# nianticlabs/acezero

Hardware: AMD Instinct MI355X
Metric: ACE patches/sec (higher is better)
Workload: dtype bf16; 1 GPU; 7-Scenes-chess-like ace_zero mapping step: 8M-patch bf16 feature buffer in HBM, batch 5120 per GPU, default head (1 block, 2 103 300 params), tanh loss, 1cyclepoly AdamW, pose_refinement none; buffer_patches=8000000, batch_per_gpu=5120, global_batch=5120, parallelism=dp1

## Files before the change

acezero_amd/csrc/head_api.hip:

```cpp
#include "head_kernels.hip"
#include "pose_fused.hip"
#include "head_maps.hip"
#include "acez_common.h"
#include "conv_launch.h"
#include <stdlib.h>
#include <string.h>
#include <algorithm>
#include "acez_common.h"
#include <vector>
#include <new>

using namespace acez;

struct StepCarry {
  bool wave_pending = false;
  const int64_t* idx = nullptr;
  int n = 0;
  bool in_alt = false;
  void hold(const int64_t* i, int k, bool alt) { idx = i; n = k; in_alt = alt; }
  void drop_batch() { hold(nullptr, 0, false); }
};

struct acez_trainer {
  char* arena_base = nullptr;
// ... 33 lines not shown
  TrainState* st_infer = nullptr;
  hipStream_t pose_stream = nullptr;
  hipEvent_t ev_begin = nullptr, ev_pose_fwd = nullptr, ev_loss = nullptr, ev_pose_bwd = nullptr;
  GradReduceArgs last_reduce{};
  StepCarry carry;
  SchedConfig sc;
  std::vector<void*> allocs;
  int pose_images = 0;
  float *pa1 = nullptr, *pa2 = nullptr, *pa3 = nullptr, *pr = nullptr, *pf1 = nullptr, *pf2 = nullptr, *pdlt = nullptr, *pose_cur = nullptr;
  float *pdT = nullptr, *pddelta = nullptr, *pdz2 = nullptr, *pdz1 = nullptr, *pdr = nullptr, *pdzc3 = nullptr, *pdzc2 = nullptr, *pdzc1 = nullptr;
  float* pose_wt = nullptr;
  bool pose_fused = true;
  int pose_tile = 4;
  bool pose_wt_valid = false;
  float* row_dT = nullptr;
  int* row_image = nullptr;
  bool profiling = false;
  std::vector<hipEvent_t> ev_pool;
  struct EvUse { int cls, i0, i1, launches; };
  std::vector<EvUse> ev_used;
  size_t ev_next = 0;
  int prof_launches = 0;
  bool seq = true;
  bool f16 = false;
  int last_nblk = 0;
  int n_cus = 0;
  uint32_t* seq_flags = nullptr;
  uint32_t seq_base[64] = {};
  uint32_t* seq_xcc = nullptr;
  int* seq_err = nullptr;
  uint32_t seq_spin_limit = 40000;
  int seq_faults = 0;
  int seq_probe = -1;
  long seq_launches = 0, seq_fault_at = -1;
  bool wgrad_opt = true;
  float* wg_xch = nullptr;
  uint32_t* wg_flags = nullptr;
  uint32_t wg_epoch = 0;
  uint16_t* R0_alt = nullptr;
  int4* batch_meta_alt = nullptr;
  long wgo_fault_at = -1;
  int wgo_fault_mod = 0;
  uint32_t* wg_status = nullptr;
  WgoFaultRec* wg_rec = nullptr;
  int wgo_recovered = 0;
  bool inference_only = false;
  bool sizing = false;
  size_t sized_total = 0;
  unsigned long long* pose_trace = nullptr;
  unsigned long long* wgo_trace = nullptr;
};

enum { KC_SCHED = 0, KC_GATHER, KC_GEMM_FWD, KC_LOSS, KC_GEMM_DGRAD, KC_WGRAD, KC_REDUCE, KC_ADAMW, KC_COUNT };

static int loss_blocks(int n) { return (n + 15) / 16; }
static int gather_blocks(int n) { return (n + 3) / 4 < 1024 ? (n + 3) / 4 : 1024; }

template <class F>
static void with_pose_tile(const acez_trainer* tr, int n_images, F f) {
  if (tr->pose_tile == 16) f(std::integral_constant<int, 16>{}, (n_images + 15) / 16);
  else f(std::integral_constant<int, 4>{}, (n_images + 3) / 4);
}

struct ProfScope {
  acez_trainer* tr; hipStream_t s; int cls; int i0 = -1;
  ProfScope(acez_trainer* t, hipStream_t st, int c) : tr(t), s(st), cls(c) {
// ... 130 lines not shown
  ACEZ_REQUIRE(cfg->schedule >= 0 && cfg->schedule <= 2, "unknown schedule");
  ACEZ_REQUIRE(cfg->loss_type >= 0 && cfg->loss_type <= 4, "unknown loss type");
  ACEZ_REQUIRE(cfg->pose_refinement >= 0 && cfg->pose_refinement <= 2, "pose_refinement must be 0 (none), 1 (naive) or 2 (mlp)");
  ACEZ_REQUIRE(cfg->pose_refinement_ortho == 0 || cfg->pose_refinement_ortho == 1, "pose_refinement_ortho must be 0 (gram-schmidt) or 1 (procrustes)");
  ACEZ_REQUIRE(cfg->pose_refinement == 0 || (params->d_pose_params && params->d_pose_m && params->d_pose_v), "pose refinement needs the pose parameter buffers");
  ACEZ_REQUIRE(cfg->pose_refinement != 2 || params->n_pose_params == ACEZ_POSE_MLP_PARAMS, "mlp: n_pose_params must be ACEZ_POSE_MLP_PARAMS");
  ACEZ_REQUIRE(cfg->pose_refinement != 1 || (params->n_pose_params > 0 && params->n_pose_params % 12 == 0), "naive: n_pose_params must be 12 * n_images");
  ACEZ_REQUIRE(cfg->compute_dtype != ACEZ_DTYPE_FP32, "compute_dtype fp32 (train_ace.py --use_half False) is not implemented: choose ACEZ_DTYPE_BF16 or ACEZ_DTYPE_FP16");
  ACEZ_REQUIRE(cfg->compute_dtype == ACEZ_DTYPE_BF16 || cfg->compute_dtype == ACEZ_DTYPE_FP16, "unknown compute_dtype");
  if (int rc = acez::require_device("the head kernels need a gfx950 GPU")) return rc;
  if (device >= 0) ACEZ_HIP_CHECK(hipSetDevice(device));
  acez_trainer* tr = new (std::nothrow) acez_trainer();
  ACEZ_REQUIRE(tr, "out of host memory");
  ACEZ_HIP_CHECK(hipGetDevice(&tr->device));
  tr->cfg = *cfg;
  tr->f16 = cfg->compute_dtype == ACEZ_DTYPE_FP16;
  if (const char* e = ACEZ_DIAG_ENV("ACEZ_POSE_FUSED")) tr->pose_fused = atoi(e) != 0;
  if (const char* e = ACEZ_DIAG_ENV("ACEZ_POSE_TILE")) tr->pose_tile = atoi(e) == 16 ? 16 : 4;
  if (cfg->pose_refinement != 2) tr->pose_fused = false;
  if (cfg->pose_refinement != 0 && !tr->pose_fused) {
    ACEZ_HIP_CHECK(hipStreamCreateWithFlags(&tr->pose_stream, hipStreamNonBlocking));
    for (hipEvent_t* e : {&tr->ev_begin, &tr->ev_pose_fwd, &tr->ev_loss, &tr->ev_pose_bwd}) ACEZ_HIP_CHECK(hipEventCreateWithFlags(e, hipEventDisableTiming));
  }
  tr->pb = *params;
  tr->nb = cfg->head.num_head_blocks;
  tr->L = 3 + 3 * tr->nb + 2;
  tr->no = cfg->head.use_homogeneous ? 4 : 3;
  tr->n_wide = (int64_t)tr->L * (512 * 512 + 512);
  tr->fc3_off = tr->n_wide;
  tr->n_params = params->n_params;
  tr->fc3_stride = ((int64_t)tr->no * 513 + 3) & ~3LL;
  tr->max_batch = cfg->max_batch;
  if (const char* e = getenv("ACEZ_SEQ")) tr->seq = atoi(e) != 0;
  {
    hipDeviceProp_t prop;
    ACEZ_HIP_CHECK(hipGetDeviceProperties(&prop, tr->device));
    tr->n_cus = prop.multiProcessorCount;
  }
  tr->nslabs = 256 / (16 * tr->L);
  if (tr->nslabs < 1) tr->nslabs = 1;

  int rc = ACEZ_OK;
  const size_t act_bytes = (size_t)tr->max_batch * 512 * sizeof(uint16_t);
  auto A = [&](void** p, size_t bytes) { if (rc == ACEZ_OK) rc = dmalloc(tr, p, bytes); };
  const bool trains = cfg->inference_only == 0;
  tr->inference_only = !trains;
  const int wgo_grid = 256 * ((tr->L + 7) / 8);
  for (int pass = 0; pass < 2; ++pass) {
  tr->sizing = pass == 0;
  A((void**)&tr->Wb, (size_t)tr->L * 262144 * 2);
  A((void**)&tr->WbT, (size_t)tr->L * 262144 * 2);
  A((void**)&tr->W3b, (size_t)tr->no * 512 * 2);
  tr->out.resize(tr->L, nullptr);
  tr->dZ.resize(tr->L, nullptr);
  tr->R.resize(tr->nb + 2, nullptr);
  for (int l = 0; l < tr->L; ++l) { A((void**)&tr->out[l], act_bytes); if (trains) A((void**)&tr->dZ[l], act_bytes); }
  for (int b = 0; b < tr->nb + 2; ++b) A((void**)&tr->R[b], act_bytes);
  const int max_loss_blocks = loss_blocks(tr->max_batch);
  tr->bias_layer_stride = (int64_t)max_loss_blocks * 512;
  if (trains) {
    A((void**)&tr->dR[0], act_bytes);
    A((void**)&tr->dR[1], act_bytes);
    tr->mask_stride = (size_t)((tr->max_batch + 79) / 80) * 4 * 4 * 64;
    A((void**)&tr->maskbits, (size_t)tr->L * tr->mask_stride * sizeof(uint2));
    A((void**)&tr->slabs, (size_t)tr->nslabs * tr->n_wide * sizeof(float));
    A((void**)&tr->fc3_partials, (size_t)max_loss_blocks * tr->fc3_stride * sizeof(float));
// ... 123 lines not shown
  a.Wb = tr->Wb; a.WbT = tr->WbT; a.W3b = tr->W3b;
  for (int l = 0; l < tr->L; ++l) { a.w_off[l] = (int64_t)l * 262656; a.b_off[l] = a.w_off[l] + 262144; }
  a.fc3_off = tr->fc3_off; a.n_fc3 = (int64_t)tr->no * 513; a.n_params = tr->n_params;
  a.n_layers = tr->L; a.no = tr->no; a.st = tr->st;
  a.slabs = nullptr; a.nslabs = 0; a.slab_stride = 0;
  a.fault = tr->seq_err; a.f16 = tr->f16 ? 1 : 0;
  a.layer_lo = 0; a.layer_hi = tr->L;
}

extern "C" int acez_trainer_sync_weights(acez_trainer* tr, void* stream) {
  ACEZ_REQUIRE(tr, "null trainer");
  ACEZ_HIP_CHECK(hipSetDevice(tr->device));
  AdamArgs a;
  fill_adam_args(tr, a);
  const int nblk = tr->L * 64 + (tr->no * 512 + 255) / 256;
  hipLaunchKernelGGL(recast_kernel, dim3(nblk), dim3(256), 0, (hipStream_t)stream, a);
  ACEZ_HIP_CHECK(hipGetLastError());
  tr->pose_wt_valid = false;
  tr->carry.drop_batch();
  return ACEZ_OK;
}

static bool seq_usable(const acez_trainer* tr, int n) {
  const int mtiles = (n + 79) / 80;
  return tr->seq && mtiles <= 64 && 32 * ((mtiles + 7) / 8) <= tr->n_cus;
}

static bool wgrad_opt_usable(const acez_trainer* tr) {
  return tr->wgrad_opt && tr->seq && tr->nslabs == 2 &&
         tr->cfg.pose_refinement == 0 && 256 * ((tr->L + 7) / 8) <= tr->n_cus;
}

template <bool BWD>
static void launch_rowseq(acez_trainer* tr, const std::vector<SeqLayer>& layers, int n, const TrainState* st, hipStream_t s) {
  const int mtiles = (n + 79) / 80;
  for (size_t i0 = 0; i0 < layers.size(); i0 += SEQ_MAX_LAYERS) {
    RowSeqArgs a{};
    const int cnt = (int)std::min<size_t>(SEQ_MAX_LAYERS, layers.size() - i0);
    for (int i = 0; i < cnt; ++i) a.layer[i] = layers[i0 + i];
    a.n_layers = cnt; a.M = n; a.st = st ? st : tr->st_infer; a.flags = tr->seq_flags; a.xcc_dbg = tr->seq_xcc; a.spin_limit = tr->seq_spin_limit;
    for (int mt = 0; mt < 64; ++mt) a.base[mt] = tr->seq_base[mt];
    if (cnt > 1 && tr->seq_launches == tr->seq_fault_at)
      for (int mt = 0; mt < 64; ++mt) a.base[mt] += 1u << 20;
    ++tr->seq_launches;
    if (tr->f16) hipLaunchKernelGGL((rowseq_kernel<BWD, EltF16>), dim3(32 * ((mtiles + 7) / 8)), dim3(512), 0, s, a);
    else hipLaunchKernelGGL(rowseq_kernel<BWD>, dim3(32 * ((mtiles + 7) / 8)), dim3(512), 0, s, a);
    for (int mt = 0; mt < mtiles; ++mt) tr->seq_base[mt] += (uint32_t)(cnt - 1);
    tr->prof_launches += cnt;
  }
}

static uint16_t* launch_forward(acez_trainer* tr, const uint16_t* in0, int n, const TrainState* st, hipStream_t s,
                                std::vector<SeqLayer>* collect = nullptr) {
  ProfScope chain_scope(tr, s, collect ? -1 : KC_GEMM_FWD);
  const float* P = tr->pb.d_params;
  const bool seq = collect || seq_usable(tr, n);
  std::vector<SeqLayer> sq;
  auto mask_out = [&](int l) -> uint2* { return (st && tr->maskbits && l != 3 * (tr->nb + 1) + 1) ? tr->maskbits + (size_t)l * tr->mask_stride : nullptr; };
  auto gemm = [&](int l, const uint16_t* in, uint16_t* out_main, const uint16_t* res, uint16_t* out_aux) {
    if (seq) {
      SeqLayer y{};
      y.In = in; y.W = tr->Wb + (size_t)l * 262144; y.bias = P + (int64_t)l * 262656 + 262144; y.res = res; y.out_main = out_main;
      y.out_aux = out_aux; y.aux_mode = res ? AUX_RESIDUAL : AUX_NONE;
      y.mask_out = mask_out(l);
      sq.push_back(y);
      return;
    }
    RowGemmArgs g{};
    g.In = in; g.W = tr->Wb + (size_t)l * 262144; g.bias = P + (int64_t)l * 262656 + 262144;
    g.add = nullptr; g.mask_out = mask_out(l); g.mask_in = nullptr; g.res = res; g.out_main = out_main; g.out_aux = out_aux;
    g.M = n; g.N = 512; g.K = 512; g.relu = 1; g.aux_mode = res ? AUX_RESIDUAL : AUX_NONE; g.st = st; g.bias_partials = nullptr;
    launch_rowgemm(g, s, tr->f16);
    ++tr->prof_launches;
  };
  const uint16_t* r = in0;
  for (int b = 0; b <= tr->nb; ++b) {
    gemm(3 * b, r, tr->out[3 * b], nullptr, nullptr);
    gemm(3 * b + 1, tr->out[3 * b], tr->out[3 * b + 1], nullptr, nullptr);
    gemm(3 * b + 2, tr->out[3 * b + 1], mask_out(3 * b + 2) ? nullptr : tr->out[3 * b + 2], r, tr->R[b + 1]);
    r = tr->R[b + 1];
// ... 95 lines not shown
}

static void fill_wgrad_args(acez_trainer* tr, WgradArgs& a, int n, const TrainState* st) {
  const int f1 = 3 * (tr->nb + 1), f2 = f1 + 1;
  for (int l = 0; l < tr->L; ++l) {
    a.dZ[l] = tr->dZ[l];
    a.w_off[l] = (int64_t)l * 262656; a.b_off[l] = a.w_off[l] + 262144;
  }
  for (int b = 0; b <= tr->nb; ++b) {
    a.In[3 * b] = tr->R[b]; a.In[3 * b + 1] = tr->out[3 * b]; a.In[3 * b + 2] = tr->out[3 * b + 1];
  }
  a.In[f1] = tr->R[tr->nb + 1]; a.In[f2] = tr->out[f1];
  a.slabs = tr->slabs; a.slab_stride = tr->n_wide; a.M = n; a.nslabs = tr->nslabs; a.n_layers = tr->L; a.st = st; a.zeros = tr->zeros;
}


enum class Flow { Fused, Backward, Update };
enum class Opt { None, WgradOpt, AdamwPose, AdamwNext, AdamwSplitPose, Adamw };
enum class NextAt { None, Loss, Optimiser };

struct StepPlan {
  Flow flow;
  bool begin_launch = false, begin_gathers = false, begin_pose = false;
  NextAt next_at = NextAt::None;
  Opt opt = Opt::None;
};

struct StepRun {
  acez_trainer* tr;
  StepPlan plan;
  const int64_t* idx; int n;
  const int64_t* next; int n_next;
  int nblk;
  hipStream_t s, ps;
  const TrainState* st;
};

static StepPlan plan_step(const acez_trainer* tr, Flow flow, const int64_t* idx, int n, const int64_t* next, int n_next) {
  StepPlan p{flow};
  const bool pf = tr->pose_fused, announced = next && n_next > 0;
  if (flow != Flow::Update) {
    const StepCarry& c = tr->carry;
    const bool have = !c.in_alt && c.idx == idx && c.n == n;
    p.begin_gathers = !have || (!pf && c.wave_pending);
    p.begin_pose = pf;
    p.begin_launch = p.begin_gathers || pf;
    if (flow == Flow::Backward) return p;
  }
  if (flow == Flow::Fused && wgrad_opt_usable(tr)) p.opt = Opt::WgradOpt;
  else if (flow == Flow::Fused && pf) p.opt = Opt::AdamwPose;
  else if (announced && tr->cfg.pose_refinement == 0 && tr->have_buf) p.opt = Opt::AdamwNext;
  else if (tr->cfg.pose_refinement != 0) p.opt = Opt::AdamwSplitPose;
  else p.opt = Opt::Adamw;
  if (announced && (p.opt == Opt::WgradOpt || p.opt == Opt::AdamwPose)) p.next_at = NextAt::Loss;
  else if (p.opt == Opt::AdamwNext || (announced && p.opt == Opt::AdamwSplitPose && pf && tr->have_buf)) p.next_at = NextAt::Optimiser;
  return p;
}

static void wave_ran(acez_trainer* tr) {
  tr->st_cur ^= 1;
  tr->st = tr->st_slot[tr->st_cur];
  tr->carry.wave_pending = false;
}

static void flush_post(acez_trainer* tr, hipStream_t s) {
  if (!tr->carry.wave_pending) return;
// ... 23 lines not shown
  else if (wave)
    hipLaunchKernelGGL(step_begin_kernel, dim3(gblocks + 1), dim3(256), 0, s, (const uint16_t*)tr->buf.d_features, d_indices, tr->R[0], n,
                       post_args(tr), gather_meta(tr));
  else
    hipLaunchKernelGGL(gather_kernel, dim3(gblocks), dim3(256), 0, s, (const uint16_t*)tr->buf.d_features, d_indices, tr->R[0], n, (const TrainState*)tr->st,
                       gather_meta(tr));
  if (wave) wave_ran(tr);
}

static void close_step(acez_trainer* tr, const StepPlan& p) {
  if (tr->carry.in_alt) {
    std::swap(tr->R[0], tr->R0_alt);
    std::swap(tr->batch_meta, tr->batch_meta_alt);
    tr->carry.in_alt = false;
  }
  if (p.opt != Opt::WgradOpt && p.opt != Opt::AdamwNext) tr->carry.wave_pending = true;
}

static void launch_train_loss(const StepRun& r) {
  acez_trainer* tr = r.tr;
  LossArgs a{};
  fill_loss_train(tr, a, tr->out[3 * (tr->nb + 1) + 1], r.idx, r.n, tr->cfg.pose_refinement != 0);
  tr->last_nblk = r.nblk;
  ProfScope ps(tr, r.s, KC_LOSS);
  if (r.plan.next_at != NextAt::Loss) return launch_loss(tr, r.nblk, r.s, a);
  const int gblocks = std::min((r.n_next + 31) / 32, std::max(32, 2 * tr->n_cus - r.nblk));
  GatherMeta gm = gather_meta(tr);
  gm.dst = tr->batch_meta_alt;
  if (tr->f16) hipLaunchKernelGGL((loss_gather_kernel<EltF16, 4>), dim3(r.nblk + gblocks), dim3(256), 0, r.s, a, r.nblk, (const uint16_t*)tr->buf.d_features, r.next, tr->R0_alt, r.n_next, gm);
  else hipLaunchKernelGGL((loss_gather_kernel<EltBf16, 4>), dim3(r.nblk + gblocks), dim3(256), 0, r.s, a, r.nblk, (const uint16_t*)tr->buf.d_features, r.next, tr->R0_alt, r.n_next, gm);
  tr->carry.hold(r.next, r.n_next, true);
}

static void launch_dgrad(acez_trainer* tr, int n, const TrainState* st, hipStream_t s, std::vector<SeqLayer>* collect = nullptr) {
  const int f1 = 3 * (tr->nb + 1), f2 = f1 + 1;
  const bool seq = collect || seq_usable(tr, n);
  std::vector<SeqLayer> sq;
  auto dgrad = [&](int l, int l_out, const uint16_t* add, uint16_t* out_main, uint16_t* out_aux) {
    const uint2* mask = tr->maskbits + (size_t)l_out * tr->mask_stride;
    if (seq) {
      if (add && !out_aux) abort();
      SeqLayer y{};
      y.In = tr->dZ[l]; y.W = tr->WbT + (size_t)l * 262144; y.add = add; y.mask_in = mask; y.out_main = out_main; y.out_aux = out_aux;
      y.bias_partials = tr->bias_partials + (size_t)l_out * tr->bias_layer_stride; y.aux_mode = out_aux ? AUX_UNMASKED : AUX_NONE;
      sq.push_back(y);
      return;
    }
    RowGemmArgs g{};
    g.bias_partials = tr->bias_partials + (size_t)l_out * tr->bias_layer_stride;
    g.In = tr->dZ[l]; g.W = tr->WbT + (size_t)l * 262144; g.bias = nullptr; g.add = add; g.mask_in = mask; g.mask_out = nullptr; g.res = nullptr;
    g.out_main = out_main; g.out_aux = out_aux; g.M = n; g.N = 512; g.K = 512; g.relu = 0;
    g.aux_mode = out_aux ? AUX_UNMASKED : AUX_NONE; g.st = st;
    g.absmax = tr->f16 ? tr->st->dz_absmax_slots : nullptr;
    launch_rowgemm(g, s, tr->f16);
    ++tr->prof_launches;
  };
  ProfScope dchain(tr, s, collect ? -1 : KC_GEMM_DGRAD);
  dgrad(f2, f1, nullptr, tr->dZ[f1], nullptr);
  int cur = 0;
  dgrad(f1, 3 * tr->nb + 2, nullptr, tr->dZ[3 * tr->nb + 2], tr->dR[cur]);
  for (int b = tr->nb; b >= 0; --b) {
    dgrad(3 * b + 2, 3 * b + 1, nullptr, tr->dZ[3 * b + 1], nullptr);
    dgrad(3 * b + 1, 3 * b, nullptr, tr->dZ[3 * b], nullptr);
    if (b > 0) {
      dgrad(3 * b, 3 * (b - 1) + 2, tr->dR[cur], tr->dZ[3 * (b - 1) + 2], tr->dR[cur ^ 1]);
      cur ^= 1;
    }
  }
  if (collect) *collect = sq;
  else if (seq) launch_rowseq<true>(tr, sq, n, st, s);
}

static void launch_weight_grads(acez_trainer* tr, const StepPlan& p, int n, int nblk, const TrainState* st, hipStream_t s) {
  const bool fused = p.flow == Flow::Fused;
  const int f2 = 3 * (tr->nb + 1) + 1;
  {
    GradReduceArgs a{};
    a.slabs = tr->slabs; a.slab_stride = tr->n_wide; a.nslabs = tr->nslabs; a.fc3_partials = tr->fc3_partials;
    a.fc3_stride = tr->fc3_stride; a.stat_partials = tr->stat_partials; a.n_loss_blocks = nblk; a.grad = tr->pb.d_grad;
    a.n_wide = tr->n_wide; a.n_params = tr->n_params; a.st = st;
    a.bias_partials = tr->bias_partials; a.bias_layer_stride = tr->bias_layer_stride; a.n_layers = tr->L;
    a.skip_wide = fused ? 1 : 0;
    a.fault = tr->seq_err;
    for (int l = 0; l < tr->L; ++l) a.bias_count[l] = (l == f2) ? nblk : (n + 79) / 80;
    tr->last_reduce = a;
  }
  {
    WgradArgs a{};
    fill_wgrad_args(tr, a, n, st);
    ProfScope ps(tr, s, KC_WGRAD);
    const int groups = tr->L * tr->nslabs;
    if (p.opt == Opt::WgradOpt) {
      WgradOptArgs o{};
      fill_adam_args(tr, o.ad);
      o.ad.tail = tr->last_reduce;
      o.xch = tr->wg_xch; o.flags = tr->wg_flags; o.spin_limit = tr->seq_spin_limit;
      o.trace = tr->wgo_trace;
      o.target = 2u * ++tr->wg_epoch;
      o.epoch = tr->wg_epoch; o.status = tr->wg_status; o.rec = tr->wg_rec;
      if ((long)tr->wg_epoch - 1 == tr->wgo_fault_at) {
        if (tr->wgo_fault_mod > 0) o.fault_mod = tr->wgo_fault_mod;
        else o.target += 1u << 20;
      }
// ... 68 lines not shown
  }
  default: {
    ProfScope ps(tr, s, KC_ADAMW);
    hipLaunchKernelGGL(adamw_kernel, dim3(n_adam), dim3(256), 0, s, a);
    break;
  }
  }
  close_step(tr, p);
  ACEZ_HIP_CHECK(hipGetLastError());
  return ACEZ_OK;
}

static void pose_fwd_launches(acez_trainer* tr, hipStream_t q) {
  if (tr->cfg.pose_refinement == 2) pose_forward(tr, &tr->st->active, q);
  if (tr->cfg.pose_refinement == 1)
    hipLaunchKernelGGL(pose_compose_kernel, dim3((tr->buf.n_images + 255) / 256), dim3(256), 0, q, (const float*)tr->pa1,
                       (const float*)tr->pb.d_pose_params, 1.0f, tr->pose_cur, tr->buf.n_images, (const int*)&tr->st->active, tr->cfg.pose_refinement_ortho);
}
static void pose_bwd_launches(acez_trainer* tr, int n, hipStream_t q) {
  if (tr->cfg.pose_refinement == 0) return;
  const int I = tr->buf.n_images;
  const int* active = &tr->st->active;
  hipLaunchKernelGGL(pose_grad_reduce2_kernel, dim3((I + 15) / 16), dim3(256), 0, q, (const float*)tr->row_dT, (const int*)tr->row_image, n, tr->pdT, I, active);
  if (tr->cfg.pose_refinement == 2) {
    hipLaunchKernelGGL(pose_mlp_bwd_kernel, dim3((I + PN_IMG - 1) / PN_IMG), dim3(256), 0, q, pose_net_args(tr, active));
    launch_pose_wgrad(tr, active, false, q);
  } else {
    hipLaunchKernelGGL(pose_compose_bwd_kernel, dim3((I + 255) / 256), dim3(256), 0, q, (const float*)tr->pa1, (const float*)tr->pb.d_pose_params, 1.0f,
                       (const float*)tr->pdT, tr->pb.d_grad + tr->n_params + 4, I, active, tr->cfg.pose_refinement_ortho);
  }
}

static StepRun start_run(acez_trainer* tr, Flow flow, const int64_t* idx, int n, const int64_t* next, int n_next, hipStream_t s) {
  return StepRun{tr, plan_step(tr, flow, idx, n, next, n_next), idx, n, next, n_next, loss_blocks(n), s, tr->pose_stream ? tr->pose_stream : s, nullptr};
}

static void launch_chain(const StepRun& r, bool bwd) {
  if (bwd) launch_dgrad(r.tr, r.n, r.st, r.s);
  else launch_forward(r.tr, r.tr->R[0], r.n, r.st, r.s);
}

template <class Chains>
static int run_steps(StepRun* runs, int count, Chains chains) {
  for (int i = 0; i < count; ++i) {
    StepRun& r = runs[i];
    acez_trainer* tr = r.tr;
    tr->last_n = r.n;
    begin_step(tr, r.plan, r.idx, r.n, r.s);
    r.st = tr->st;
    if (r.ps != r.s) {
      ACEZ_HIP_CHECK(hipEventRecord(tr->ev_begin, r.s));
      ACEZ_HIP_CHECK(hipStreamWaitEvent(r.ps, tr->ev_begin, 0));
    }
    if (!tr->pose_fused) pose_fwd_launches(tr, r.ps);
    if (r.ps != r.s) ACEZ_HIP_CHECK(hipEventRecord(tr->ev_pose_fwd, r.ps));
  }
  chains(false);
  for (int i = 0; i < count; ++i) {
    StepRun& r = runs[i];
    acez_trainer* tr = r.tr;
    if (r.ps != r.s) ACEZ_HIP_CHECK(hipStreamWaitEvent(r.s, tr->ev_pose_fwd, 0));
    launch_train_loss(r);
    if (r.ps != r.s) {
      ACEZ_HIP_CHECK(hipEventRecord(tr->ev_loss, r.s));
      ACEZ_HIP_CHECK(hipStreamWaitEvent(r.ps, tr->ev_loss, 0));
    }
    if (!tr->pose_fused) pose_bwd_launches(tr, r.n, r.ps);
    if (r.ps != r.s) ACEZ_HIP_CHECK(hipEventRecord(tr->ev_pose_bwd, r.ps));
  }
  chains(true);
  for (int i = 0; i < count; ++i) {
    StepRun& r = runs[i];
    acez_trainer* tr = r.tr;
    launch_weight_grads(tr, r.plan, r.n, r.nblk, r.st, r.s);
    if (r.ps != r.s) ACEZ_HIP_CHECK(hipStreamWaitEvent(r.s, tr->ev_pose_bwd, 0));
    if (tr->pose_fused && r.plan.flow == Flow::Backward) launch_pose_wgrad(tr, &tr->st->active, false, r.s);
    ACEZ_HIP_CHECK(hipGetLastError());
    if (r.plan.flow == Flow::Fused) {
      const int rc = launch_update(tr, r.plan, r.s, 0, tr->L, r.next, r.n_next);
      if (rc != ACEZ_OK) return rc;
    }
  }
  return ACEZ_OK;
}

static int train_step_impl(acez_trainer* tr, Flow flow, const int64_t* d_indices, int n, void* stream, const int64_t* d_next = nullptr, int n_next = 0) {
  ACEZ_REQUIRE(tr && d_indices, "null pointer");
  ACEZ_REQUIRE(!tr->inference_only, "an inference-only context (acez_train_config.inference_only) cannot train");
  ACEZ_REQUIRE(tr->have_buf, "acez_trainer_set_buffer has not been called");
  ACEZ_REQUIRE(n > 0 && n <= tr->max_batch, "n must be in [1, max_batch]");
  ACEZ_HIP_CHECK(hipSetDevice(tr->device));
  StepRun r = start_run(tr, flow, d_indices, n, d_next, n_next, (hipStream_t)stream);
  return run_steps(&r, 1, [&](bool bwd) { launch_chain(r, bwd); });
}

extern "C" int acez_train_backward(acez_trainer* tr, const int64_t* d_indices, int n, void* stream) {
  return train_step_impl(tr, Flow::Backward, d_indices, n, stream);
}

static int train_update_impl(acez_trainer* tr, void* stream, int layer_lo, int layer_hi, const int64_t* d_next = nullptr, int n_next = 0) {
  ACEZ_REQUIRE(tr, "null trainer");
  ACEZ_REQUIRE(!tr->inference_only, "an inference-only context (acez_train_config.inference_only) cannot train");
  if (layer_hi < 0) layer_hi = tr->L;
  ACEZ_REQUIRE(layer_lo >= 0 && layer_lo <= layer_hi && layer_hi <= tr->L, "layer range out of bounds");
  ACEZ_HIP_CHECK(hipSetDevice(tr->device));
  return launch_update(tr, plan_step(tr, Flow::Update, nullptr, 0, d_next, n_next), (hipStream_t)stream, layer_lo, layer_hi, d_next, n_next);
}

extern "C" int acez_train_update(acez_trainer* tr, void* stream) { return train_update_impl(tr, stream, 0, -1); }
extern "C" int acez_train_update_next(acez_trainer* tr, const int64_t* d_indices_next, int n_next, void* stream) {
  ACEZ_REQUIRE(n_next >= 0 && (!tr || n_next <= tr->max_batch), "n_next must be in [0, max_batch]");
  return train_update_impl(tr, stream, 0, -1, d_indices_next, n_next);
}

extern "C" int acez_train_update_layers(acez_trainer* tr, int layer_lo, int layer_hi, void* stream) {
  return train_update_impl(tr, stream, layer_lo, layer_hi);
}

extern "C" int acez_trainer_export_weights16(acez_trainer* tr, int layer_lo, int layer_hi, void* d_dst, void* stream) {
  ACEZ_REQUIRE(tr && d_dst, "null pointer");
  ACEZ_REQUIRE(layer_lo >= 0 && layer_lo <= layer_hi && layer_hi <= tr->L, "layer range out of bounds");
  if (layer_hi == layer_lo) return ACEZ_OK;
  ACEZ_HIP_CHECK(hipSetDevice(tr->device));
  ACEZ_HIP_CHECK(hipMemcpyAsync(d_dst, tr->Wb + (size_t)layer_lo * 262144, (size_t)(layer_hi - layer_lo) * 262144 * 2, hipMemcpyDeviceToDevice, (hipStream_t)stream));
  return ACEZ_OK;
// ... 230 lines not shown
```

acezero_amd/csrc/head_kernels.hip:

```cpp
#include <hip/hip_runtime.h>
#include <stdint.h>
#include "head_kernels.h"
#include "gemm_common.h"

namespace acez {


template <int GR = 4>
__device__ __forceinline__ void gather_rows(const uint16_t* __restrict__ feat, const int64_t* __restrict__ idx, uint16_t* __restrict__ out, int n,
                                            int wave, int nwaves, int lane, const GatherMeta& meta) {
  const bool held = meta.hold && *meta.hold;
  for (int r0 = wave; r0 < n; r0 += GR * nwaves) {
    int r[GR];
    bool ok[GR];
    int64_t s[GR];
#pragma unroll
    for (int j = 0; j < GR; ++j) { r[j] = r0 + j * nwaves; ok[j] = r[j] < n; s[j] = idx[ok[j] ? r[j] : r0]; }
    uint4 v[GR];
#pragma unroll
    for (int j = 0; j < GR; ++j) v[j] = *reinterpret_cast<const uint4*>(feat + s[j] * 512 + lane * 8);
    int view[GR];
    float2 tp[GR];
    if (meta.dst) {
#pragma unroll
// ... 380 lines not shown
template <bool BIAS_RELU, bool HAS_ADD, bool HAS_MASK, int AUX, class E = EltBf16>
__global__ __launch_bounds__(512) void rowgemm80_kernel(RowGemmArgs a) {
  const int active = a.st ? a.st->active : 1;
  __shared__ __attribute__((aligned(16))) uint16_t smem[RG80_SMEM];
  const int mtiles = (a.M + 79) / 80;
  const int per_xcd = (mtiles + 7) >> 3;
  const int jx = blockIdx.x >> 3;
  const int mt = (blockIdx.x & 7) * per_xcd + (jx >> 2);
  if (mt >= mtiles) return;
  rowgemm80_body<BIAS_RELU, HAS_ADD, HAS_MASK, AUX, false, E>(a, smem, active, mt, (jx & 3) * 128, SeqLink{});
}

struct SeqLayer {
  const uint16_t *In, *W;
  const float* bias;
  const uint16_t *add, *res;
  uint2* mask_out;
  const uint2* mask_in;
  uint16_t *out_main, *out_aux;
  float* bias_partials;
  int aux_mode, pad;
};
constexpr int SEQ_MAX_LAYERS = 8;
struct RowSeqArgs {
  SeqLayer layer[SEQ_MAX_LAYERS];
  int n_layers, M;
  const TrainState* st;
  uint32_t* flags;
  uint32_t base[64];
  uint32_t spin_limit;
  uint32_t* xcc_dbg;
};

template <bool BWD, class E = EltBf16>
__global__ __launch_bounds__(512) void rowseq_kernel(RowSeqArgs a) {
  __shared__ __attribute__((aligned(16))) uint16_t smem[RG80_SMEM_SEQ];
  const int mtiles = (a.M + 79) / 80;
  const int per_xcd = (mtiles + 7) >> 3;
  const int jx = blockIdx.x >> 3;
  const int mt = (blockIdx.x & 7) * per_xcd + (jx >> 2);
  if (mt >= mtiles) return;
  if (a.xcc_dbg && threadIdx.x == 0) {
    const uint32_t xcc = __builtin_amdgcn_s_getreg((3 << 11) | 20) & 15u;
    atomicOr(a.xcc_dbg + (blockIdx.x & 7), 1u << xcc);
    a.xcc_dbg[8 + mt * 4 + (jx & 3)] = xcc;
  }
  if ((a.st && !a.st->active) || a.flags[64 * 32]) {
    if (threadIdx.x == 0) {
      const uint32_t inc = 8u * (uint32_t)(a.n_layers - 1);
      asm volatile("global_atomic_add %0, %1, off" ::"v"(a.flags + mt * 32), "v"(inc) : "memory");
    }
    return;
  }
  const int n0 = (jx & 3) * 128;
  for (int layer = 0; layer < a.n_layers; ++layer) {
    const SeqLayer& y = a.layer[layer];
    RowGemmArgs g;
    g.In = y.In; g.W = y.W; g.bias = y.bias; g.add = y.add; g.mask_out = y.mask_out; g.mask_in = y.mask_in; g.res = y.res; g.out_main = y.out_main; g.out_aux = y.out_aux;
    g.bias_partials = y.bias_partials; g.M = a.M; g.N = 512; g.K = 512; g.relu = BWD ? 0 : 1; g.aux_mode = y.aux_mode; g.st = a.st;
    g.absmax = (BWD && a.st) ? const_cast<uint32_t*>(a.st->dz_absmax_slots) : nullptr;
    SeqLink q;
    q.flag = a.flags + mt * 32; q.target = (a.base[mt] + (uint32_t)layer) * 32u;
    q.first = layer == 0; q.wait = layer > 0; q.signal = layer + 1 < a.n_layers;
    q.next_W = q.signal ? a.layer[layer + 1].W : nullptr;
    q.flag_index = (uint32_t)(mt * 32); q.limit = a.spin_limit;
    if (!BWD) {
      if (y.aux_mode == AUX_RESIDUAL) rowgemm80_body<true, false, false, AUX_RESIDUAL, true, E>(g, smem, 1, mt, n0, q);
      else rowgemm80_body<true, false, false, AUX_NONE, true, E>(g, smem, 1, mt, n0, q);
    } else {
      if (y.add) rowgemm80_body<false, true, true, AUX_UNMASKED, true, E>(g, smem, 1, mt, n0, q);
      else if (y.aux_mode == AUX_UNMASKED) rowgemm80_body<false, false, true, AUX_UNMASKED, true, E>(g, smem, 1, mt, n0, q);
      else rowgemm80_body<false, false, true, AUX_NONE, true, E>(g, smem, 1, mt, n0, q);
    }
  }
}

__global__ __launch_bounds__(512) void seq_probe_kernel(uint32_t* rec , int mtiles) {
  __shared__ __attribute__((aligned(16))) uint16_t smem[RG80_SMEM_SEQ];
  const int per_xcd = (mtiles + 7) >> 3;
  const int jx = blockIdx.x >> 3;
  const int mt = (blockIdx.x & 7) * per_xcd + (jx >> 2);
  if (threadIdx.x == 0) smem[0] = (uint16_t)blockIdx.x;
  __syncthreads();
  if (mt >= mtiles || threadIdx.x != 0) return;
  const uint32_t xcc = __builtin_amdgcn_s_getreg((3 << 11) | 20) & 15u;
  rec[mt * 4 + (jx & 3)] = (xcc << 16) | smem[0];
}

static inline void launch_rowgemm(const RowGemmArgs& g, hipStream_t s, bool f16 = false) {
  const bool br = g.bias != nullptr;
  const int mtiles = (g.M + 79) / 80;
  const dim3 grid(8 * 4 * ((mtiles + 7) / 8));
#define ACEZ_RG(...)                                                                                               \
  do {                                                                                                             \
    if (f16) hipLaunchKernelGGL((rowgemm80_kernel<__VA_ARGS__, EltF16>), grid, dim3(512), 0, s, g);                \
    else hipLaunchKernelGGL((rowgemm80_kernel<__VA_ARGS__>), grid, dim3(512), 0, s, g);                            \
  } while (0)
  if (br && g.aux_mode == AUX_NONE) ACEZ_RG(true, false, false, AUX_NONE);
  else if (br && g.aux_mode == AUX_RESIDUAL) ACEZ_RG(true, false, false, AUX_RESIDUAL);
  else if (!br && g.mask_in && !g.add && g.aux_mode == AUX_NONE) ACEZ_RG(false, false, true, AUX_NONE);
  else if (!br && g.mask_in && !g.add && g.aux_mode == AUX_UNMASKED) ACEZ_RG(false, false, true, AUX_UNMASKED);
  else if (!br && g.mask_in && g.add && g.aux_mode == AUX_UNMASKED) ACEZ_RG(false, true, true, AUX_UNMASKED);
  else if (!br && g.mask_in && g.add && g.aux_mode == AUX_NONE) ACEZ_RG(false, true, true, AUX_NONE);
  else abort();
#undef ACEZ_RG
}

// ... 1222 lines not shown
    if (threadIdx.x < 64) {
      if (a.slabs) {
        sched_post_wave(p.src, p.st, p.c, p.grad_stats, p.inv_global_batch, p.log_loss, p.log_inl, p.log_cap, p.fault, p.stat_partials, p.n_loss_blocks, &a.tail);
      } else {
        sched_post_wave(p.src, p.st, p.c, p.grad_stats, p.inv_global_batch, p.log_loss, p.log_inl, p.log_cap, p.fault, p.stat_partials, p.n_loss_blocks);
      }
    }
    return;
  }
  adamw_body(a, b - gblocks - 1, tileT);
}

__device__ double det_cos_pi(double x) {
  const double PI = 3.14159265358979323846;
  const double y = (x - 0.5) * PI;
  const double y2 = y * y;
  double term = y, sum = y;
  for (int k = 1; k <= 11; ++k) {
    term = -term * y2 / (double)((2 * k) * (2 * k + 1));
    sum += term;
  }
  return -sum;
}

constexpr int WGO_PF = 17;
__device__ __forceinline__ void lds_wait_ge(uint32_t* f, uint32_t target) {
  while (__hip_atomic_load(f, __ATOMIC_RELAXED, __HIP_MEMORY_SCOPE_WORKGROUP) < target) __builtin_amdgcn_s_sleep(1);
  asm volatile("" ::: "memory");
}
__device__ __forceinline__ void lds_bump(uint32_t* f) {
  asm volatile("s_waitcnt lgkmcnt(0)" ::: "memory");
  if ((threadIdx.x & 63) == 0) __hip_atomic_fetch_add(f, 1u, __ATOMIC_RELAXED, __HIP_MEMORY_SCOPE_WORKGROUP);
}
#ifdef ACEZ_DIAG
#define WGO_STAMP(i) do { if (o.trace && (threadIdx.x & 63) == 0) o.trace[((size_t)blockIdx.x * 12 + (threadIdx.x >> 6)) * 8 + (i)] = __builtin_amdgcn_s_memtime(); } while (0)
#else
#define WGO_STAMP(i) do { } while (0)
#endif
template <class E = EltBf16>
__global__ __launch_bounds__(WGRAD_THREADS) void wgrad_opt_kernel(WgradArgs a, WgradOptArgs o, PostArgs post) {
  constexpr int RING = WGRAD_RING;
  static_assert(RING >= 3, "two free ring slots are used as staging areas after the K loop");
  __shared__ __attribute__((aligned(16))) uint16_t smem[RING][2][64 * 128];
  __shared__ uint32_t wsync[2];
  const int t = threadIdx.x, l = t & 63;
  const int w = __builtin_amdgcn_readfirstlane(t >> 6);
  const int b = blockIdx.x;
  const int xcd = b & 7, jx = b >> 3;
  const int layer = xcd + 8 * (jx >> 5), slab = (jx >> 4) & 1, tile = jx & 15;
  if (layer >= a.n_layers) return;
  if (t < 2) wsync[t] = 0;
  WGO_STAMP(0);
  const int n0 = (tile >> 2) * 128, c0 = (tile & 3) * 128;
  const AdamArgs& ad = o.ad;
  const int e = t - 256, rb = e >> 5, col4 = (e & 31) * 4;
  const int64_t woff = ad.w_off[layer];
  const int nrow0 = n0 + 64 * slab;
  float4 p4[4], m4[4], v4[4];
  float lp[5];
  uint32_t amx = 0u, amxm = 0u;
  const int nlb = ad.tail.n_loss_blocks;
  auto prefetch = [&]() {
#pragma unroll
    for (int i = 0; i < 4; ++i) {
      const int64_t off = woff + (int64_t)(nrow0 + rb + 16 * i) * 512 + c0 + col4;
      p4[i] = *reinterpret_cast<const float4*>(ad.params + off);
// ... 222 lines not shown
```

Baseline: 36.20 million patches/s.

## Fuse training loss and next-batch gather into the backward row-sequence chain kernel

Adds a rowseq_loss_kernel that computes the tanh loss per M-tile, gathers the next batch's features, and then signals the sequential dgrad chain through the existing per-tile flags. This replaces the separate loss launch and the kernel boundary before the backward GEMM chain. Weights for the first backward layer are prefetched into LDS while the loss runs. It is enabled by default when wgrad_opt and the seq path apply, and can be disabled through an environment variable. The cost is more complex flag bookkeeping and extra spin-wait coupling between the loss and GEMM stages.

```diff
diff --git a/acezero_amd/csrc/head_api.hip b/acezero_amd/csrc/head_api.hip
--- a/acezero_amd/csrc/head_api.hip
+++ b/acezero_amd/csrc/head_api.hip
@@ -89,6 +89,7 @@
   uint32_t seq_spin_limit = 40000;
   int seq_faults = 0;
   int seq_probe = -1;
+  bool loss_in_chain = true;
   long seq_launches = 0, seq_fault_at = -1;
   bool wgrad_opt = true;
   float* wg_xch = nullptr;
@@ -285,6 +286,7 @@
   tr->fc3_stride = ((int64_t)tr->no * 513 + 3) & ~3LL;
   tr->max_batch = cfg->max_batch;
   if (const char* e = getenv("ACEZ_SEQ")) tr->seq = atoi(e) != 0;
+  if (const char* e = getenv("ACEZ_LOSS_IN_CHAIN")) tr->loss_in_chain = atoi(e) != 0;
   {
     hipDeviceProp_t prop;
     ACEZ_HIP_CHECK(hipGetDeviceProperties(&prop, tr->device));
@@ -474,20 +476,26 @@
 }
 
 template <bool BWD>
-static void launch_rowseq(acez_trainer* tr, const std::vector<SeqLayer>& layers, int n, const TrainState* st, hipStream_t s) {
+static void launch_rowseq(acez_trainer* tr, const std::vector<SeqLayer>& layers, int n, const TrainState* st, hipStream_t s,
+                          const SeqLossArgs* head = nullptr) {
   const int mtiles = (n + 79) / 80;
   for (size_t i0 = 0; i0 < layers.size(); i0 += SEQ_MAX_LAYERS) {
+    const bool with_loss = BWD && head && i0 == 0;
     RowSeqArgs a{};
     const int cnt = (int)std::min<size_t>(SEQ_MAX_LAYERS, layers.size() - i0);
     for (int i = 0; i < cnt; ++i) a.layer[i] = layers[i0 + i];
     a.n_layers = cnt; a.M = n; a.st = st ? st : tr->st_infer; a.flags = tr->seq_flags; a.xcc_dbg = tr->seq_xcc; a.spin_limit = tr->seq_spin_limit;
     for (int mt = 0; mt < 64; ++mt) a.base[mt] = tr->seq_base[mt];
-    if (cnt > 1 && tr->seq_launches == tr->seq_fault_at)
+    if ((cnt > 1 || with_loss) && tr->seq_launches == tr->seq_fault_at)
       for (int mt = 0; mt < 64; ++mt) a.base[mt] += 1u << 20;
     ++tr->seq_launches;
-    if (tr->f16) hipLaunchKernelGGL((rowseq_kernel<BWD, EltF16>), dim3(32 * ((mtiles + 7) / 8)), dim3(512), 0, s, a);
+    if (with_loss) {
+      if (tr->f16) hipLaunchKernelGGL(rowseq_loss_kernel<EltF16>, dim3(32 * ((mtiles + 7) / 8)), dim3(512), 0, s, a, *head);
+      else hipLaunchKernelGGL(rowseq_loss_kernel<EltBf16>, dim3(32 * ((mtiles + 7) / 8)), dim3(512), 0, s, a, *head);
+    }
+    else if (tr->f16) hipLaunchKernelGGL((rowseq_kernel<BWD, EltF16>), dim3(32 * ((mtiles + 7) / 8)), dim3(512), 0, s, a);
     else hipLaunchKernelGGL(rowseq_kernel<BWD>, dim3(32 * ((mtiles + 7) / 8)), dim3(512), 0, s, a);
-    for (int mt = 0; mt < mtiles; ++mt) tr->seq_base[mt] += (uint32_t)(cnt - 1);
+    for (int mt = 0; mt < mtiles; ++mt) tr->seq_base[mt] += (uint32_t)(cnt - 1 + (with_loss ? 1 : 0));
     tr->prof_launches += cnt;
   }
 }
@@ -649,6 +657,7 @@
   const int64_t* idx; int n;
   const int64_t* next; int n_next;
   int nblk;
+  bool loss_in_chain = false;
   hipStream_t s, ps;
   const TrainState* st;
 };
@@ -738,7 +747,23 @@
   tr->carry.hold(r.next, r.n_next, true);
 }
 
-static void launch_dgrad(acez_trainer* tr, int n, const TrainState* st, hipStream_t s, std::vector<SeqLayer>* collect = nullptr) {
+static SeqLossArgs train_loss_in_chain(const StepRun& r) {
+  acez_trainer* tr = r.tr;
+  SeqLossArgs x{};
+  fill_loss_train(tr, x.loss, tr->out[3 * (tr->nb + 1) + 1], r.idx, r.n, false);
+  x.nblk = r.nblk;
+  tr->last_nblk = r.nblk;
+  if (r.plan.next_at == NextAt::Loss) {
+    x.feat = (const uint16_t*)tr->buf.d_features; x.idx_next = r.next; x.out_next = tr->R0_alt; x.n_next = r.n_next;
+    x.meta = gather_meta(tr);
+    x.meta.dst = tr->batch_meta_alt;
+    tr->carry.hold(r.next, r.n_next, true);
+  }
+  return x;
+}
+
+static void launch_dgrad(acez_trainer* tr, int n, const TrainState* st, hipStream_t s, std::vector<SeqLayer>* collect = nullptr,
+                         const StepRun* inchain = nullptr) {
   const int f1 = 3 * (tr->nb + 1), f2 = f1 + 1;
   const bool seq = collect || seq_usable(tr, n);
   std::vector<SeqLayer> sq;
@@ -774,7 +799,12 @@
     }
   }
   if (collect) *collect = sq;
+  else if (seq && inchain) {
+    const SeqLossArgs x = train_loss_in_chain(*inchain);
+    launch_rowseq<true>(tr, sq, n, st, s, &x);
+  }
   else if (seq) launch_rowseq<true>(tr, sq, n, st, s);
+  else if (inchain) abort();
 }
 
 static void launch_weight_grads(acez_trainer* tr, const StepPlan& p, int n, int nblk, const TrainState* st, hipStream_t s) {
@@ -909,11 +939,11 @@
 }
 
 static StepRun start_run(acez_trainer* tr, Flow flow, const int64_t* idx, int n, const int64_t* next, int n_next, hipStream_t s) {
-  return StepRun{tr, plan_step(tr, flow, idx, n, next, n_next), idx, n, next, n_next, loss_blocks(n), s, tr->pose_stream ? tr->pose_stream : s, nullptr};
+  return StepRun{tr, plan_step(tr, flow, idx, n, next, n_next), idx, n, next, n_next, loss_blocks(n), false, s, tr->pose_stream ? tr->pose_stream : s, nullptr};
 }
 
 static void launch_chain(const StepRun& r, bool bwd) {
-  if (bwd) launch_dgrad(r.tr, r.n, r.st, r.s);
+  if (bwd) launch_dgrad(r.tr, r.n, r.st, r.s, nullptr, r.loss_in_chain ? &r : nullptr);
   else launch_forward(r.tr, r.tr->R[0], r.n, r.st, r.s);
 }
 
@@ -937,7 +967,7 @@
     StepRun& r = runs[i];
     acez_trainer* tr = r.tr;
     if (r.ps != r.s) ACEZ_HIP_CHECK(hipStreamWaitEvent(r.s, tr->ev_pose_fwd, 0));
-    launch_train_loss(r);
+    if (!r.loss_in_chain) launch_train_loss(r);
     if (r.ps != r.s) {
       ACEZ_HIP_CHECK(hipEventRecord(tr->ev_loss, r.s));
       ACEZ_HIP_CHECK(hipStreamWaitEvent(r.ps, tr->ev_loss, 0));
@@ -968,6 +998,7 @@
   ACEZ_REQUIRE(n > 0 && n <= tr->max_batch, "n must be in [1, max_batch]");
   ACEZ_HIP_CHECK(hipSetDevice(tr->device));
   StepRun r = start_run(tr, flow, d_indices, n, d_next, n_next, (hipStream_t)stream);
+  r.loss_in_chain = tr->loss_in_chain && r.plan.opt == Opt::WgradOpt && seq_usable(tr, n);
   return run_steps(&r, 1, [&](bool bwd) { launch_chain(r, bwd); });
 }
 
diff --git a/acezero_amd/csrc/head_kernels.hip b/acezero_amd/csrc/head_kernels.hip
--- a/acezero_amd/csrc/head_kernels.hip
+++ b/acezero_amd/csrc/head_kernels.hip
@@ -436,6 +436,30 @@
   uint32_t* xcc_dbg;
 };
 
+template <bool BWD, class E, int SEAM0>
+__device__ __forceinline__ void rowseq_layers(const RowSeqArgs& a, uint16_t* smem, const int mt, const int n0) {
+  for (int layer = 0; layer < a.n_layers; ++layer) {
+    const SeqLayer& y = a.layer[layer];
+    RowGemmArgs g;
+    g.In = y.In; g.W = y.W; g.bias = y.bias; g.add = y.add; g.mask_out = y.mask_out; g.mask_in = y.mask_in; g.res = y.res; g.out_main = y.out_main; g.out_aux = y.out_aux;
+    g.bias_partials = y.bias_partials; g.M = a.M; g.N = 512; g.K = 512; g.relu = BWD ? 0 : 1; g.aux_mode = y.aux_mode; g.st = a.st;
+    g.absmax = (BWD && a.st) ? const_cast<uint32_t*>(a.st->dz_absmax_slots) : nullptr;
+    SeqLink q;
+    q.flag = a.flags + mt * 32; q.target = (a.base[mt] + (uint32_t)(layer + SEAM0)) * 32u;
+    q.first = !SEAM0 && layer == 0; q.wait = SEAM0 || layer > 0; q.signal = layer + 1 < a.n_layers;
+    q.next_W = q.signal ? a.layer[layer + 1].W : nullptr;
+    q.flag_index = (uint32_t)(mt * 32); q.limit = a.spin_limit;
+    if (!BWD) {
+      if (y.aux_mode == AUX_RESIDUAL) rowgemm80_body<true, false, false, AUX_RESIDUAL, true, E>(g, smem, 1, mt, n0, q);
+      else rowgemm80_body<true, false, false, AUX_NONE, true, E>(g, smem, 1, mt, n0, q);
+    } else {
+      if (y.add) rowgemm80_body<false, true, true, AUX_UNMASKED, true, E>(g, smem, 1, mt, n0, q);
+      else if (y.aux_mode == AUX_UNMASKED) rowgemm80_body<false, false, true, AUX_UNMASKED, true, E>(g, smem, 1, mt, n0, q);
+      else rowgemm80_body<false, false, true, AUX_NONE, true, E>(g, smem, 1, mt, n0, q);
+    }
+  }
+}
+
 template <bool BWD, class E = EltBf16>
 __global__ __launch_bounds__(512) void rowseq_kernel(RowSeqArgs a) {
   __shared__ __attribute__((aligned(16))) uint16_t smem[RG80_SMEM_SEQ];
@@ -456,27 +480,7 @@
     }
     return;
   }
-  const int n0 = (jx & 3) * 128;
-  for (int layer = 0; layer < a.n_layers; ++layer) {
-    const SeqLayer& y = a.layer[layer];
-    RowGemmArgs g;
-    g.In = y.In; g.W = y.W; g.bias = y.bias; g.add = y.add; g.mask_out = y.mask_out; g.mask_in = y.mask_in; g.res = y.res; g.out_main = y.out_main; g.out_aux = y.out_aux;
-    g.bias_partials = y.bias_partials; g.M = a.M; g.N = 512; g.K = 512; g.relu = BWD ? 0 : 1; g.aux_mode = y.aux_mode; g.st = a.st;
-    g.absmax = (BWD && a.st) ? const_cast<uint32_t*>(a.st->dz_absmax_slots) : nullptr;
-    SeqLink q;
-    q.flag = a.flags + mt * 32; q.target = (a.base[mt] + (uint32_t)layer) * 32u;
-    q.first = layer == 0; q.wait = layer > 0; q.signal = layer + 1 < a.n_layers;
-    q.next_W = q.signal ? a.layer[layer + 1].W : nullptr;
-    q.flag_index = (uint32_t)(mt * 32); q.limit = a.spin_limit;
-    if (!BWD) {
-      if (y.aux_mode == AUX_RESIDUAL) rowgemm80_body<true, false, false, AUX_RESIDUAL, true, E>(g, smem, 1, mt, n0, q);
-      else rowgemm80_body<true, false, false, AUX_NONE, true, E>(g, smem, 1, mt, n0, q);
-    } else {
-      if (y.add) rowgemm80_body<false, true, true, AUX_UNMASKED, true, E>(g, smem, 1, mt, n0, q);
-      else if (y.aux_mode == AUX_UNMASKED) rowgemm80_body<false, false, true, AUX_UNMASKED, true, E>(g, smem, 1, mt, n0, q);
-      else rowgemm80_body<false, false, true, AUX_NONE, true, E>(g, smem, 1, mt, n0, q);
-    }
-  }
+  rowseq_layers<BWD, E, 0>(a, smem, mt, (jx & 3) * 128);
 }
 
 __global__ __launch_bounds__(512) void seq_probe_kernel(uint32_t* rec , int mtiles) {
@@ -1765,6 +1769,76 @@
   asm volatile("s_waitcnt lgkmcnt(0)" ::: "memory");
   if ((threadIdx.x & 63) == 0) __hip_atomic_fetch_add(f, 1u, __ATOMIC_RELAXED, __HIP_MEMORY_SCOPE_WORKGROUP);
 }
+
+struct SeqLossArgs {
+  LossArgs loss;
+  int nblk;
+  const uint16_t* feat;
+  const int64_t* idx_next;
+  uint16_t* out_next;
+  int n_next;
+  GatherMeta meta;
+};
+
+template <class E = EltBf16>
+__global__ __launch_bounds__(512) void rowseq_loss_kernel(RowSeqArgs a, SeqLossArgs x) {
+  __shared__ __attribute__((aligned(16))) uint16_t smem[RG80_SMEM_SEQ];
+  const int mtiles = (a.M + 79) / 80;
+  const int per_xcd = (mtiles + 7) >> 3;
+  const int jx = blockIdx.x >> 3;
+  const int mt = (blockIdx.x & 7) * per_xcd + (jx >> 2);
+  if (mt >= mtiles) return;
+  const int t = threadIdx.x, l = t & 63;
+  const int w = __builtin_amdgcn_readfirstlane(t >> 6);
+  const int nt = jx & 3, n0 = nt * 128;
+  if (a.xcc_dbg && t == 0) {
+    const uint32_t xcc = __builtin_amdgcn_s_getreg((3 << 11) | 20) & 15u;
+    atomicOr(a.xcc_dbg + (blockIdx.x & 7), 1u << xcc);
+    a.xcc_dbg[8 + mt * 4 + nt] = xcc;
+  }
+  uint32_t* const qsync = reinterpret_cast<uint32_t*>(smem + RG80_SMEM);
+  if (t < 2) qsync[t] = 0u;
+  asm volatile("s_waitcnt lgkmcnt(0)" ::: "memory");
+  __builtin_amdgcn_s_barrier();
+  const bool dead = (a.st && !a.st->active) || a.flags[64 * 32];
+  if (w >= 4) {
+    const int lw = w - 4;
+    if (!dead) {
+#pragma unroll
+      for (int j = 0; j < 4; ++j) {
+        const int row = (lw * 4 + j) * 8 + (l >> 3);
+        const uint16_t* g = a.layer[0].W + (size_t)(n0 + row) * 512 + ((l & 7) ^ ((row >> 1) & 7)) * 8;
+#pragma unroll
+        for (int kt = 0; kt < 4; ++kt)
+          __builtin_amdgcn_global_load_lds((gvoid_t*)(g + kt * 64), (lvoid_t*)(smem + kt * RG80_STAGE + (lw * 4 + j) * 8 * 64), 16, 0, 0);
+      }
+    }
+    if (nt != 0 && x.n_next > 0) gather_rows<8>(x.feat, x.idx_next, x.out_next, x.n_next, (mt * 3 + nt - 1) * 4 + lw, mtiles * 12, l, x.meta);
+  }
+  if (dead) {
+    if (t == 0) {
+      const uint32_t inc = 8u * (uint32_t)a.n_layers;
+      asm volatile("global_atomic_add %0, %1, off" ::"v"(a.flags + mt * 32), "v"(inc) : "memory");
+    }
+    return;
+  }
+  if (w < 4 || nt == 0) {
+    const int quartet = w >> 2;
+    const int block = 5 * mt + (nt == 0 ? quartet : nt + 1);
+    if (block < x.nblk) {
+      float* scratch = reinterpret_cast<float*>(smem + 4 * RG80_STAGE) + quartet * (3 * 4 * 4 * 4);
+      uint32_t* const f = qsync + quartet;
+      loss_body<false, true, E, 4>(x.loss, block, w & 3, l, nullptr, scratch, LossPre{0, 0, 0, 0.f, 0.f}, [f] { lds_bump(f); lds_wait_ge(f, 4u); });
+    }
+    ACEZ_VMCNT(0);
+    if (l == 0) {
+      const uint32_t inc = nt == 0 ? 1u : 2u;
+      asm volatile("global_atomic_add %0, %1, off" ::"v"(a.flags + mt * 32), "v"(inc) : "memory");
+    }
+  }
+  rowseq_layers<true, E, 1>(a, smem, mt, n0);
+}
+
 #ifdef ACEZ_DIAG
 #define WGO_STAMP(i) do { if (o.trace && (threadIdx.x & 63) == 0) o.trace[((size_t)blockIdx.x * 12 + (threadIdx.x >> 6)) * 8 + (i)] = __builtin_amdgcn_s_memtime(); } while (0)
 #else
```

Measured after the change: 37.19 million patches/s, median of 6. +2.7%, better.
